# manikya7022/Continual-Learning-for-Dynamic-Video-Quality-Enhancement

Measured on AMD Instinct MI355X. Metric: train frames/sec (2x SR, T=3, 540p->1080p), higher is better.
Workload: dtype bf16

## Files before the change

### continual-learning-for-dynamic-video-quality-enhancement_amd/csrc/conv_bf16.hip

```cpp
#include "conv_common.h"

namespace nvq {

#ifdef NVQ_DEBUG_TOOLS
static int g_debug_mode = 0;
void set_conv_debug_mode(int m) { g_debug_mode = m; }
#else
constexpr int g_debug_mode = 0;
#endif

constexpr int XSB = 48;

__device__ __forceinline__ __bf16 pack_bf16_elem(const float* __restrict__ w, int cout_w, int cin_w, int taps, int transpose,
                                                 int cout_keep, int NT, int nkc, long idx) {
    const int stride = ws_stride_halfs(taps, NT);
    long t = idx % stride;
    const long slab = idx / stride;
    if (t >= (long)taps * 4 * NT * 8) return (__bf16)0.f;
    const int j = t & 7; t >>= 3;
    const int n = t % NT; t /= NT;
    const int g = t & 3; t >>= 2;
    const int tap = (int)t;
    const int kc = slab % nkc;
    const int cz = (int)(slab / nkc);
    const int co = cz * NT + n;
    const int ch = kc * KCB + 8 * g + j;
    float v = 0.f;
    if (!transpose) {
        if (co < cout_w && ch < cin_w) v = w[((long)co * cin_w + ch) * taps + tap];
    } else {
        if (co < cout_keep && ch < cout_w) v = w[((long)ch * cin_w + co) * taps + (taps - 1 - tap)];
    }
    return (__bf16)v;
}

__global__ void pack_bf16_kernel(const float* __restrict__ w, int cout_w, int cin_w, int taps, int transpose,
                                 int cout_keep, int NT, int ncz, int nkc, __bf16* __restrict__ wp) {
    const long total = (long)ncz * nkc * ws_stride_halfs(taps, NT);
    for (long idx = blockIdx.x * (long)blockDim.x + threadIdx.x; idx < total; idx += (long)gridDim.x * blockDim.x)
        wp[idx] = pack_bf16_elem(w, cout_w, cin_w, taps, transpose, cout_keep, NT, nkc, idx);
}

__global__ void pack_batch_bf16_kernel(const PackJobTable t) {
    const PackJobDev j = t.j[blockIdx.y];
    __bf16* wp = reinterpret_cast<__bf16*>(j.wp);
    for (long idx = blockIdx.x * (long)blockDim.x + threadIdx.x; idx < j.total; idx += (long)gridDim.x * blockDim.x)
        wp[idx] = pack_bf16_elem(j.w, j.cout_w, j.cin_w, j.taps, j.transpose, j.cout_keep, j.NT, j.nkc, idx);
}

struct TailArgs {
    const float* frames;
    float* out;
    unsigned char* pass;
    int T, t_center, Cimg;
};
__device__ __forceinline__ float tcc1(float x) { const float A = -0.75f; return ((A + 2.f) * x - (A + 3.f)) * x * x + 1.f; }
__device__ __forceinline__ float tcc2(float x) { const float A = -0.75f; return ((A * x - 5.f * A) * x + 8.f * A) * x - 4.f * A; }
__device__ __forceinline__ void tail_cubic_taps(int dst, float scale, int size, int idx[4], float w[4]) {
    const float real = scale * ((float)dst + 0.5f) - 0.5f;
    const float fl = floorf(real);
    const float t = real - fl;
    const int i0 = (int)fl;
    w[0] = tcc2(t + 1.f);
    w[1] = tcc1(t);
    w[2] = tcc1(1.f - t);
    w[3] = tcc2((1.f - t) + 1.f);
#pragma unroll
    for (int k = 0; k < 4; ++k) idx[k] = min(max(i0 - 1 + k, 0), size - 1);
}

template <int NB, int KS, bool INB, int NW = 4, int CS = 1, int TS = 0>
__global__ __launch_bounds__(64 * NW, NW == 4 ? 2 : 4) void conv_bf16_kernel(const nvq_conv_desc d, int tilesX,
                                                                               int tilesY, int nkc, int vec_ok, int dbg,
                                                                               const TailArgs tail) {
    constexpr int NT = NB * 16;
    constexpr int NTW = NT * CS;
    constexpr int NTHR = 64 * NW;
    constexpr int TH_ = 2 * NW / CS;
    constexpr int HALO = KS / 2;
    constexpr int TAPS = KS * KS;
    constexpr int HW_ = TW + 2 * HALO;
    constexpr int HH_ = TH_ + 2 * HALO;
    constexpr int NPIX = HW_ * HH_;
    constexpr int WS_HALFS = ws_stride_halfs(TAPS, NTW);
    constexpr int XITEMS = NPIX * 4;
    constexpr int XPER = (XITEMS + NTHR - 1) / NTHR;
    constexpr int WTHR = NTHR;
    constexpr int WPIECES = TAPS * 4 * NTW;
    constexpr int WPER = (WPIECES + WTHR - 1) / WTHR;
    constexpr int XREGS = INB ? 1 : 2;
    constexpr int CT_K = (TAPS / 2) * 4 * NTW / WTHR;
    constexpr int CT_N = 4 * NTW;
    static_assert(((TAPS / 2) * 4 * NTW) % WTHR == 0 && CT_N <= 256, "the centre tap starts a WTHR-piece row");
    static_assert(CS == 1 || (CS == 2 && NW == 8 && NB == 2), "channel-split variant: 8 waves, 2 x 32 channels");

    __shared__ __attribute__((aligned(16))) __bf16 lds[NPIX * XSB + WS_HALFS];
    __bf16* xs = lds;
    __bf16* ws = lds + NPIX * XSB;
    const int kcl = KS == 3 ? d.center_cin / KCB : 0;

    const int tid = threadIdx.x;
    const int lane = tid & 63;
    const int wid = __builtin_amdgcn_readfirstlane(tid >> 6);
    const int wave = CS == 1 ? wid : wid & (NW / CS - 1);
    const int half = CS == 1 ? 0 : wid >> 2;
    const int c = lane & 15;
    const int g = lane >> 4;

    int bt = xcd_tile(blockIdx.x, gridDim.x);
    const int tx = bt % tilesX; bt /= tilesX;
    const int ty = bt % tilesY;
    const int n = bt / tilesY;
    const int cz = blockIdx.y * CS + half;
    const int H = d.h, W = d.w;

    f32x4 acc[NB][4];
#pragma unroll
    for (int a = 0; a < NB; ++a)
#pragma unroll
        for (int b = 0; b < 4; ++b) acc[a][b] = (f32x4){0.f, 0.f, 0.f, 0.f};

    const __bf16* wp_base = reinterpret_cast<const __bf16*>(d.wpack) + (size_t)blockIdx.y * nkc * WS_HALFS;
    const float* in32 = d.in + d.in_coff;
    const __bf16* in16 = reinterpret_cast<const __bf16*>(d.in) + d.in_coff;

    unsigned xoff[XPER];
    bool xok[XPER];
#pragma unroll
    for (int k = 0; k < XPER; ++k) {
        const int item = tid + k * NTHR;
        const int hp = item >> 2;
        const int hy = hp / HW_, hx = hp - hy * HW_;
        const int gy = ty * TH_ + hy - HALO, gx = tx * TW + hx - HALO;
        xok[k] = item < XITEMS && gy >= 0 && gy < H && gx >= 0 && gx < W;
        xoff[k] = xok[k] ? (unsigned)(((size_t)(n * H + gy) * W + gx) * (d.in_plane ? 32 : d.in_ld)) : 0u;
    }
    const int nk0 = d.in_plane ? d.in_ld >> 5 : 0x7fffffff;
    const int sh0 = d.in_plane ? __ffs(d.in_ld >> 5) - 1 : 0;
    const bool interior = ty * TH_ >= HALO && tx * TW >= HALO && ty * TH_ + TH_ + HALO <= H && tx * TW + TW + HALO <= W &&
                          d.cin % KCB == 0;
    const int chg = 8 * (tid & 3);
    u32x4 xr[XPER][XREGS];
    u32x4 wr[WPER];

    bool cv0 = false, cv1 = false;
    auto fetch = [&](int kc, bool light) {
        const int ch = kc * KCB + chg;
        cv0 = ch < d.cin;
        cv1 = ch + 4 < d.cin;
        const bool lead = kc < nk0;
        const int sh = lead ? sh0 : 0;
        const unsigned cbase = lead ? (unsigned)kc * KCB : (unsigned)kc * d.in_plane;
        const unsigned o0 = cv0 ? cbase + chg : 0u, o1 = cv1 ? cbase + chg + 4 : 0u;
#pragma unroll
        for (int k = 0; k < XPER; ++k) {
            if constexpr (INB) {
                xr[k][0] = *reinterpret_cast<const u32x4*>(in16 + ((xoff[k] << sh) + o0));
            } else {
                xr[k][0] = *reinterpret_cast<const u32x4*>(in32 + ((xoff[k] << sh) + o0));
                xr[k][XREGS - 1] = *reinterpret_cast<const u32x4*>(in32 + ((xoff[k] << sh) + o1));
            }
        }
        const u32x4* wsrc = reinterpret_cast<const u32x4*>(wp_base + (size_t)kc * WS_HALFS);
        if (light) {
            wr[CT_K] = wsrc[(tid < CT_N ? tid : 0) + CT_K * WTHR];
        } else {
#pragma unroll
            for (int k = 0; k < WPER; ++k) wr[k] = wsrc[tid + k * WTHR < WPIECES ? tid + k * WTHR : 0];
        }
    };
    auto commit = [&](int kc, bool light) {
        const u32x4 z = {0u, 0u, 0u, 0u};
        if (interior) {
#pragma unroll
            for (int k = 0; k < XPER; ++k) {
                const int item = tid + k * NTHR;
                if (item < XITEMS) {
                    __bf16* dst = xs + (item >> 2) * XSB + 8 * (item & 3);
                    if constexpr (INB) *reinterpret_cast<u32x4*>(dst) = xr[k][0];
                    else *reinterpret_cast<bf16x8*>(dst) = cvt8(as_f4(xr[k][0]), as_f4(xr[k][XREGS - 1]));
                }
            }
        } else {
#pragma unroll
            for (int k = 0; k < XPER; ++k) {
                const int item = tid + k * NTHR;
                const bool v0 = xok[k] && cv0, v1 = xok[k] && cv1;
                if (item < XITEMS) {
                    __bf16* dst = xs + (item >> 2) * XSB + 8 * (item & 3);
                    if constexpr (INB)
                        *reinterpret_cast<u32x4*>(dst) = v0 ? xr[k][0] : z;
                    else
                        *reinterpret_cast<bf16x8*>(dst) = cvt8(as_f4(v0 ? xr[k][0] : z), as_f4(v1 ? xr[k][XREGS - 1] : z));
                }
            }
        }
        if (light) {
            if (tid < CT_N) reinterpret_cast<u32x4*>(ws)[tid + CT_K * WTHR] = wr[CT_K];
        } else {
#pragma unroll
            for (int k = 0; k < WPER; ++k)
                if ((k + 1) * WTHR <= WPIECES || tid + k * WTHR < WPIECES) reinterpret_cast<u32x4*>(ws)[tid + k * WTHR] = wr[k];
        }
    };

    auto ldP = [&](int rr, int xh, int dx) -> bf16x8 {
        return *reinterpret_cast<const bf16x8*>(xs + ((2 * wave + rr) * HW_ + xh * 16 + c + dx) * XSB + 8 * g);
    };
    auto ldW = [&](int tap, int cb) -> bf16x8 {
        return *reinterpret_cast<const bf16x8*>(ws + ((tap * 4 + g) * NTW + half * NT + cb * 16 + c) * 8);
    };
    auto stage_chunk = [&](int kc, bool cl, bool fl) {
        __syncthreads();
        commit(kc, cl);
        __syncthreads();
        if (kc + 1 < nkc && !(dbg & 2)) fetch(kc + 1, fl);
    };
    auto center_stage = [&]() {
        bf16x8 p0[2], p1[2], wc[NB];
#pragma unroll
        for (int cb = 0; cb < NB; ++cb) wc[cb] = ldW(TAPS / 2, cb);
#pragma unroll
        for (int xh = 0; xh < 2; ++xh) { p0[xh] = ldP(1, xh, 1); p1[xh] = ldP(2, xh, 1); }
#pragma unroll
        for (int xh = 0; xh < 2; ++xh)
#pragma unroll
            for (int cb = 0; cb < NB; ++cb) {
                acc[cb][xh] = __builtin_amdgcn_mfma_f32_16x16x32_bf16(wc[cb], p0[xh], acc[cb][xh], 0, 0, 0);
                acc[cb][2 + xh] = __builtin_amdgcn_mfma_f32_16x16x32_bf16(wc[cb], p1[xh], acc[cb][2 + xh], 0, 0, 0);
            }
    };

    const bool dead = CS == 2 && cz * NT >= d.cout_store;
    int kc = 0;
    if constexpr (KS == 3) {
        if (kcl > 0) {
            fetch(0, true);
            for (; kc + 1 < kcl; ++kc) {
                stage_chunk(kc, true, true);
                if (!(dbg & 1) && !dead) center_stage();
            }
            stage_chunk(kc, true, false);
            if (!(dbg & 1) && !dead) center_stage();
            ++kc;
        } else {
            fetch(0, false);
        }
    } else {
        fetch(0, false);
    }
    for (; kc < nkc; ++kc) {
        stage_chunk(kc, false, false);
        if ((dbg & 1) || dead) continue;
        bf16x8 lo[2], hi[2], wa[NB], wn[NB];
        lo[0] = ldP(0, 0, 0); lo[1] = ldP(0, 1, 0);
#pragma unroll
        for (int cb = 0; cb < NB; ++cb) wa[cb] = ldW(0, cb);
        hi[0] = ldP(1, 0, 0); hi[1] = ldP(1, 1, 0);
#pragma unroll
        for (int s = 0; s < TAPS; ++s) {
            const int dy = s % KS;
            const bool last = s + 1 == TAPS;
            const int ndx = (s + 1) / KS, ndy = (s + 1) % KS;
            const bool same_dx = !last && ndy != 0;
            bf16x8 nlo[2], nhi[2];
            if (!last) {
#pragma unroll
                for (int cb = 0; cb < NB; ++cb) wn[cb] = ldW(ndy * KS + ndx, cb);
            }
#pragma unroll
            for (int xh = 0; xh < 2; ++xh) {
#pragma unroll
                for (int cb = 0; cb < NB; ++cb)
                    acc[cb][xh] = __builtin_amdgcn_mfma_f32_16x16x32_bf16(wa[cb], lo[xh], acc[cb][xh], 0, 0, 0);
                if (same_dx) nhi[xh] = ldP(dy + 2, xh, ndx);
                else if (!last) nlo[xh] = ldP(0, xh, ndx);
            }
#pragma unroll
            for (int xh = 0; xh < 2; ++xh) {
#pragma unroll
                for (int cb = 0; cb < NB; ++cb)
                    acc[cb][2 + xh] = __builtin_amdgcn_mfma_f32_16x16x32_bf16(wa[cb], hi[xh], acc[cb][2 + xh], 0, 0, 0);
                if (same_dx) nlo[xh] = hi[xh];
                else if (!last) nhi[xh] = ldP(1, xh, ndx);
            }
            if (!last) {
#pragma unroll
                for (int xh = 0; xh < 2; ++xh) { lo[xh] = nlo[xh]; hi[xh] = nhi[xh]; }
#pragma unroll
                for (int cb = 0; cb < NB; ++cb) wa[cb] = wn[cb];
            }
        }
    }
    if constexpr (TS > 0) {
        static_assert(NW == 4 && CS == 1, "8 x 32-pixel tiles");
        constexpr int CP = NT + 1;
        static_assert(TH * TW * CP * 4 <= (NPIX * XSB + WS_HALFS) * 2, "the conv output tile fits the LDS stages");
        float* ut = reinterpret_cast<float*>(lds);
        const int U = tail.Cimg * TS * TS;
        __syncthreads();
#pragma unroll
        for (int pb = 0; pb < 4; ++pb) {
            const int px = (2 * wave + (pb >> 1)) * TW + (pb & 1) * 16 + c;
#pragma unroll
            for (int cb = 0; cb < NB; ++cb)
#pragma unroll
                for (int e = 0; e < 4; ++e) {
                    const int co = cb * 16 + 4 * g + e;
                    if (co < U) ut[px * CP + co] = acc[cb][pb][e] + (d.bias ? d.bias[co] : 0.f);
                }
        }
        __syncthreads();
        const int OW = W * TS, OH = H * TS;
        const float scale = 1.f / (float)TS;
// ... 452 lines not shown
    const __bf16* r16 = reinterpret_cast<const __bf16*>(dl.res) + dl.res_coff;
    auto res_load = [&](int pb) {
        const int gy = ty * TH + 2 * w4 + (pb >> 1), gx = tx * TW + (pb & 1) * 16 + c;
        okp[pb] = gy < H && gx < W;
        const unsigned off = okp[pb] ? ((unsigned)(n * H + gy) * (unsigned)W + gx) * (unsigned)dl.res_ld + 4u * g : 0u;
#pragma unroll
        for (int cb = 0; cb < NBL; ++cb) rr[pb][cb] = *reinterpret_cast<const uint2*>(r16 + (off + cb * 16u));
    };
    if (!(dbg & 128)) { res_load(0); res_load(1); }
    __syncthreads();
    __syncthreads();
    {
        const __bf16* t4 = ws;
#pragma unroll
        for (int cb = 0; cb < NBL; ++cb) {
            const bf16x8 wf = ldL(cb);
#pragma unroll
            for (int pb = 0; pb < 4; ++pb) {
                const int px = (2 * w4 + (pb >> 1)) * TW + (pb & 1) * 16 + c;
                const bf16x8 yf = *reinterpret_cast<const bf16x8*>(t4 + px * T4S + 8 * g);
                lacc[cb][pb] = __builtin_amdgcn_mfma_f32_16x16x32_bf16(wf, yf, lacc[cb][pb], 0, 0, 0);
            }
        }
    }
    if (!(dbg & 128)) { res_load(2); res_load(3); }
#pragma unroll
    for (int cb = 0; cb < NBL; ++cb) bb[cb] = ld4(dl.bias + cb * 16 + 4 * g);
    __syncthreads();
    __bf16* stage = lds + w4 * (2 * TW * STAGE_PX64);
#pragma unroll
    for (int pb = 0; pb < 4; ++pb) {
        if (!okp[pb]) continue;
#pragma unroll
        for (int cb = 0; cb < NBL; ++cb) {
            float v[4] = {lacc[cb][pb][0] + bb[cb].x, lacc[cb][pb][1] + bb[cb].y, lacc[cb][pb][2] + bb[cb].z,
                          lacc[cb][pb][3] + bb[cb].w};
            {
#pragma clang fp contract(off)
                v[0] = v[0] * dl.alpha + __uint_as_float(rr[pb][cb].x << 16);
                v[1] = v[1] * dl.alpha + __uint_as_float(rr[pb][cb].x & 0xffff0000u);
                v[2] = v[2] * dl.alpha + __uint_as_float(rr[pb][cb].y << 16);
                v[3] = v[3] * dl.alpha + __uint_as_float(rr[pb][cb].y & 0xffff0000u);
            }
            *reinterpret_cast<bf16x4*>(stage + ((pb >> 1) * TW + (pb & 1) * 16 + c) * STAGE_PX64 + cb * 16 + 4 * g) =
                (bf16x4){(__bf16)v[0], (__bf16)v[1], (__bf16)v[2], (__bf16)v[3]};
        }
    }
    __builtin_amdgcn_fence(__ATOMIC_RELEASE, "wavefront");
    __builtin_amdgcn_wave_barrier();
    if (dbg & 16) return;
    __bf16* o16 = reinterpret_cast<__bf16*>(dl.out);
#pragma unroll
    for (int k = 0; k < 8; ++k) {
        const int item = lane + k * 64;
        const int px = item >> 3, piece = item & 7;
        const int gy = ty * TH + 2 * w4 + (px >> 5), gx = tx * TW + (px & 31);
        if (gy < H && gx < W)
            *reinterpret_cast<u32x4*>(o16 + ((size_t)(n * H + gy) * W + gx) * dl.out_ld + dl.out_coff + 8 * piece) =
                *reinterpret_cast<const u32x4*>(stage + px * STAGE_PX64 + 8 * piece);
    }
}

template <int KS, bool XB, bool YB, int CIC, int COC = 32>
__global__ __launch_bounds__(256, 2) void wgrad_bf16_kernel(const nvq_wgrad_desc d, int tilesX, int tilesY,
                                                             int ntiles, int nci32, int nco) {
    static_assert(CIC == 32 || (CIC == 64 && XB), "64-channel chunks need bf16 x");
    static_assert(COC == 32 || (COC == 64 && CIC == 64 && YB && KS == 1), "64-co chunks: 1x1, bf16 x and dy");
    constexpr int HALO = KS / 2;
    constexpr int TAPS = KS * KS;
    constexpr int HW_ = TW + 2 * HALO;
    constexpr int HH_ = TH + 2 * HALO;
    constexpr int NPIX = HW_ * HH_;
    constexpr int XSX = CIC == 64 ? 80 : XSB;
    constexpr int XPP = (XB ? 4 : 8) * (CIC / 32);
    constexpr int YSX = COC == 64 ? 80 : XSB;
    constexpr int YPP = (YB ? 4 : 8) * (COC / 32);
    constexpr int XCH = CIC / XPP, YCH = COC / YPP;
    constexpr int XITEMS = NPIX * XPP;
    constexpr int XPER = (XITEMS + 255) / 256;
    constexpr int YPER = TH * TW * YPP / 256;
    constexpr int NCO = (CIC == 64 ? 2 : 1) * (COC / 32);
    __shared__ __attribute__((aligned(16))) __bf16 lds[NPIX * XSX + TH * TW * YSX];
    __bf16* xs = lds;
    __bf16* dys = lds + NPIX * XSX;

    const int tid = threadIdx.x;
    const int lane = tid & 63;
    const int wave = tid >> 6;
    const int r = lane & 15;
    const int g = lane >> 4;
    const int q = r >> 2, p = r & 3;
    const int cib = CIC == 64 ? wave : wave >> 1;
    const int cob0 = CIC == 64 ? 0 : (wave & 1);
    const int cic = blockIdx.y, coc = blockIdx.z;
    const int H = d.h, W = d.w;
    const float* x32 = d.x + d.x_coff;
    const __bf16* x16 = reinterpret_cast<const __bf16*>(d.x) + d.x_coff;
    const float* dy32 = d.dy + d.dy_coff;
    const __bf16* dy16 = reinterpret_cast<const __bf16*>(d.dy) + d.dy_coff;

    f32x4 acc[NCO][TAPS];
#pragma unroll
    for (int a = 0; a < NCO; ++a)
#pragma unroll
        for (int t = 0; t < TAPS; ++t) acc[a][t] = (f32x4){0.f, 0.f, 0.f, 0.f};

    u32x4 xr[XPER], yr[YPER];
    float4 bsumA = make_float4(0.f, 0.f, 0.f, 0.f), bsumB = bsumA;
    const int xq = XCH * (tid & (XPP - 1));
    const int yq = YCH * (tid & (YPP - 1));
    const bool xch_ok = cic * CIC + xq < d.cin;
    const int xch = cic * CIC + xq;
    const bool xlead = !d.x_plane || xch < d.x_ld;
    const unsigned xmul = xlead ? d.x_ld : 32;
    const size_t xbase = xlead ? (size_t)xch : (size_t)(xch >> 5) * d.x_plane + (xch & 31);
    const int ych = coc * COC + yq;
    const bool ych_ok = ych < d.cout;
    unsigned xmask = 0, ymask = 0;
    auto fetch = [&](int tile) {
        int bt = xcd_tile(tile, ntiles);
        const int tx = bt % tilesX; bt /= tilesX;
        const int ty = bt % tilesY;
        const int n = bt / tilesY;
        xmask = 0; ymask = 0;
#pragma unroll
        for (int k = 0; k < XPER; ++k) {
            const int item = tid + k * 256;
            const int hp = item / XPP;
            const int hy = hp / HW_, hx = hp - hy * HW_;
            const int gy = ty * TH + hy - HALO, gx = tx * TW + hx - HALO;
            const bool ok = item < XITEMS && gy >= 0 && gy < H && gx >= 0 && gx < W && xch_ok;
            xmask |= (ok ? 1u : 0u) << k;
            const size_t off = ok ? ((size_t)(n * H + gy) * W + gx) * xmul + xbase : 0;
            if constexpr (XB) xr[k] = *reinterpret_cast<const u32x4*>(x16 + off);
            else xr[k] = *reinterpret_cast<const u32x4*>(x32 + off);
        }
#pragma unroll
        for (int k = 0; k < YPER; ++k) {
            const int item = tid + k * 256;
            const int pp = item / YPP;
            const int py = pp / TW, px = pp - py * TW;
            const int gy = ty * TH + py, gx = tx * TW + px;
            const bool ok = gy < H && gx < W && ych_ok;
            ymask |= (ok ? 1u : 0u) << k;
            const size_t off = ok ? ((size_t)(n * H + gy) * W + gx) * d.dy_ld + ych : 0;
            if constexpr (YB) yr[k] = *reinterpret_cast<const u32x4*>(dy16 + off);
            else yr[k] = *reinterpret_cast<const u32x4*>(dy32 + off);
        }
    };
    auto commit = [&]() {
        const u32x4 z = {0u, 0u, 0u, 0u};
#pragma unroll
        for (int k = 0; k < XPER; ++k) {
            const int item = tid + k * 256;
            if (item < XITEMS) {
                const u32x4 v = (xmask >> k) & 1 ? xr[k] : z;
                __bf16* dst = xs + (item / XPP) * XSX + XCH * (item & (XPP - 1));
                if constexpr (XB) *reinterpret_cast<u32x4*>(dst) = v;
                else *reinterpret_cast<bf16x4*>(dst) = cvt4(as_f4(v));
            }
        }
#pragma unroll
        for (int k = 0; k < YPER; ++k) {
            const int item = tid + k * 256;
            const u32x4 v = (ymask >> k) & 1 ? yr[k] : z;
            __bf16* dst = dys + (item / YPP) * YSX + YCH * (item & (YPP - 1));
            if constexpr (YB) {
                *reinterpret_cast<u32x4*>(dst) = v;
                bsumA.x += bf_lo(v[0]); bsumA.y += bf_hi(v[0]); bsumA.z += bf_lo(v[1]); bsumA.w += bf_hi(v[1]);
                bsumB.x += bf_lo(v[2]); bsumB.y += bf_hi(v[2]); bsumB.z += bf_lo(v[3]); bsumB.w += bf_hi(v[3]);
            } else {
                const float4 f = as_f4(v);
                *reinterpret_cast<bf16x4*>(dst) = cvt4(f);
                bsumA.x += f.x; bsumA.y += f.y; bsumA.z += f.z; bsumA.w += f.w;
            }
        }
    };
    const bool idle = cic * CIC + cib * 16 >= d.cin_w;
    typedef s16x4 __attribute__((address_space(3))) * lds_s16x4_ptr;
    auto tr_read = [&](const __bf16* base, int stride, int pix, int chblock) -> s16x4 {
        return __builtin_amdgcn_ds_read_tr16_b64_v4i16((lds_s16x4_ptr)(base + (pix + q) * stride + chblock * 16 + 4 * p));
    };

    int tile = blockIdx.x;
    if (tile < ntiles) fetch(tile);
    for (; tile < ntiles; tile += gridDim.x) {
        __syncthreads();
        commit();
        __syncthreads();
        if (tile + (int)gridDim.x < ntiles) fetch(tile + gridDim.x);
        if (idle) continue;
#pragma unroll 2
        for (int py = 0; py < TH; ++py) {
            bf16x8 bfrag[NCO];
#pragma unroll
            for (int a = 0; a < NCO; ++a) {
                const s16x4 b0 = tr_read(dys, YSX, py * TW + 4 * g, cob0 + a);
                const s16x4 b1 = tr_read(dys, YSX, py * TW + 16 + 4 * g, cob0 + a);
                bfrag[a] = __builtin_bit_cast(bf16x8, __builtin_shufflevector(b0, b1, 0, 1, 2, 3, 4, 5, 6, 7));
            }
#pragma unroll
            for (int tap = 0; tap < TAPS; ++tap) {
                const int ddy = tap / KS, ddx = tap - ddy * KS;
                const int hp = (py + ddy) * HW_ + ddx;
                const s16x4 a0 = tr_read(xs, XSX, hp + 4 * g, cib);
                const s16x4 a1 = tr_read(xs, XSX, hp + 16 + 4 * g, cib);
                const bf16x8 afrag = __builtin_bit_cast(bf16x8, __builtin_shufflevector(a0, a1, 0, 1, 2, 3, 4, 5, 6, 7));
#pragma unroll
                for (int a = 0; a < NCO; ++a)
                    acc[a][tap] = __builtin_amdgcn_mfma_f32_16x16x32_bf16(afrag, bfrag[a], acc[a][tap], 0, 0, 0);
            }
        }
    }

    const int slab = cic * (CIC / 32) + (cib * 16) / 32;
    if (slab < nci32) {
        const int cil0 = (cib * 16) % 32;
#pragma unroll
        for (int a = 0; a < NCO; ++a) {
            const int coc32 = coc * (COC / 32) + (cob0 + a) / 2, cob = (cob0 + a) % 2;
            if (coc32 >= nco) continue;
            float* part = d.workspace + ((size_t)(blockIdx.x * nci32 + slab) * nco + coc32) * (TAPS * WG_C * WG_C);
#pragma unroll
            for (int tap = 0; tap < TAPS; ++tap)
#pragma unroll
                for (int e = 0; e < 4; ++e) part[(tap * WG_C + cil0 + 4 * g + e) * WG_C + cob * 16 + r] = acc[a][tap][e];
        }
    }

    if (cic == 0 && d.dbias != nullptr) {
        float* scratch = reinterpret_cast<float*>(lds);
        __syncthreads();
        st4(scratch + 8 * tid, bsumA);
        st4(scratch + 8 * tid + 4, bsumB);
        __syncthreads();
        if (tid < COC) {
            const int piece = tid / YCH, e = tid % YCH;
            float s = 0.f;
            for (int k = 0; k < 256 / YPP; ++k) s += scratch[8 * (YPP * k + piece) + e];
            float* bp = d.workspace + (size_t)WGRAD_MAX_SLABS * 9 * WG_C * WG_C;
            const int coc32 = coc * (COC / 32) + tid / WG_C;
            if (coc32 < nco) bp[((size_t)blockIdx.x * nco + coc32) * WG_C + tid % WG_C] = s;
        }
    }
}

size_t pack_floats_bf16(int cout, int cin_store, int ksize) {
    const int NT = choose_nt(cout);
    const size_t ncz = (cout + NT - 1) / NT, nkc = (cin_store + KCB - 1) / KCB;
    return ncz * nkc * (size_t)ws_stride_halfs(ksize * ksize, NT) / 2;
}

int pack_bf16(const float* w, int cout_w, int cin_w, int ksize, int transpose, int cin_store, int cout_keep,
              float* wpack, hipStream_t s) {
    const int cout = transpose ? cout_keep : cout_w;
    const int NT = choose_nt(cout);
    const int ncz = (cout + NT - 1) / NT, nkc = (cin_store + KCB - 1) / KCB;
    const long total = (long)ncz * nkc * ws_stride_halfs(ksize * ksize, NT);
    int nblk = ceil_div(total, 256);
    if (nblk > 2048) nblk = 2048;
    hipLaunchKernelGGL(pack_bf16_kernel, dim3(nblk), dim3(256), 0, s, w, cout_w, cin_w, ksize * ksize, transpose,
                       cout_keep, NT, ncz, nkc, reinterpret_cast<__bf16*>(wpack));
    return check_launch("conv_pack_bf16");
}

PackJobDev pack_job_bf16(const nvq_pack_job& j) {
    const int cout = j.transpose ? j.cout_keep : j.cout_w;
    const int NT = choose_nt(cout);
    const int ncz = (cout + NT - 1) / NT, nkc = (j.cin_store + KCB - 1) / KCB;
    return PackJobDev{j.w, j.wpack, j.cout_w, j.cin_w, j.ksize * j.ksize, j.transpose, j.cout_keep, NT, ncz, nkc,
                      (long)ncz * nkc * ws_stride_halfs(j.ksize * j.ksize, NT)};
}

int pack_batch_bf16(const PackJobTable& t, int n, hipStream_t s) {
    hipLaunchKernelGGL(pack_batch_bf16_kernel, dim3(32, n), dim3(256), 0, s, t);
    return check_launch("conv_pack_batch(bf16)");
}

int conv_forward_bf16(const nvq_conv_desc& d, int vec_ok, hipStream_t s) {
    NVQ_REQUIRE((size_t)d.n * d.h * d.w * d.in_ld < ((size_t)1 << 32),
                "conv_forward(bf16): input tensor of %d x %d x %d x %d elements exceeds the 32-bit offsets of the kernels", d.n,
                d.h, d.w, d.in_ld);
    const int NT = choose_nt(d.cout);
    const int ncz = (d.cout_store + NT - 1) / NT;
    const int nkc = (d.cin + KCB - 1) / KCB;
    int tilesX = (d.w + TW - 1) / TW, tilesY = (d.h + TH - 1) / TH;
    const bool underfilled = tilesX * ((d.h + 2 * TH - 1) / (2 * TH)) < NVQ_SMALL_IMAGE_TILES;
    const int rows = d.tile_rows == 0 && underfilled ? 8 : d.tile_rows;
    if (d.ksize == 3 && NT == 32 && d.in_bf16 && d.h >= 2 * TH && vec_ok &&
        (rows == 162 || rows == 164 || (rows == 0 && d.cin <= 128)))
        return conv_forward_m32(d, rows == 164 ? 4 : 2, g_debug_mode & 15, s);
    if (d.ksize == 3 && NT == 32 && d.in_bf16 && d.h >= 2 * TH && rows != 8) {
        tilesY = (d.h + 2 * TH - 1) / (2 * TH);
        const dim3 grid8((unsigned)((long)tilesX * tilesY * d.n), ncz);
        hipLaunchKernelGGL((conv_bf16_kernel<2, 3, true, 8>), grid8, dim3(512), 0, s, d, tilesX, tilesY, nkc, vec_ok,
                           g_debug_mode & 3, TailArgs{});
        return check_launch("conv_forward_bf16");
    }
    if (d.ksize == 3 && NT == 64 && d.in_bf16 && (d.tile_rows == 264 || d.tile_rows == 265)) {
        NVQ_REQUIRE(vec_ok && d.out_bf16 && d.cout_store % 64 == 0 && d.cin % 8 == 0,
                    "conv_forward: tile_rows 264 / 265 need bf16 output and a multiple of 64 stored channels");
        return conv_forward_m32(d, d.tile_rows == 264 ? 64 : 65, g_debug_mode & 3, s);
    }
    if (d.ksize == 3 && NT == 64 && d.in_bf16 && d.tile_rows != 8) {
        const dim3 grid8((unsigned)((long)tilesX * tilesY * d.n), ncz);
        hipLaunchKernelGGL((conv_bf16_kernel<2, 3, true, 8, 2>), grid8, dim3(512), 0, s, d, tilesX, tilesY, nkc, vec_ok,
                           g_debug_mode & 3, TailArgs{});
        return check_launch("conv_forward_bf16");
    }
    const dim3 grid((unsigned)((long)tilesX * tilesY * d.n), ncz);
#define NVQ_LAUNCH_CONVB(NB, KS)                                                                                        \
    do {                                                                                                                 \
        if (d.in_bf16)                                                                                                   \
            hipLaunchKernelGGL((conv_bf16_kernel<NB, KS, true>), grid, dim3(256), 0, s, d, tilesX, tilesY, nkc, vec_ok, g_debug_mode & 3, TailArgs{});   \
        else                                                                                                             \
            hipLaunchKernelGGL((conv_bf16_kernel<NB, KS, false>), grid, dim3(256), 0, s, d, tilesX, tilesY, nkc, vec_ok, g_debug_mode & 3, TailArgs{});  \
    } while (0)
    if (d.ksize == 3) {
        if (NT == 16) NVQ_LAUNCH_CONVB(1, 3);
        else if (NT == 32) NVQ_LAUNCH_CONVB(2, 3);
        else NVQ_LAUNCH_CONVB(4, 3);
    } else {
        if (NT == 16) NVQ_LAUNCH_CONVB(1, 1);
        else if (NT == 32) NVQ_LAUNCH_CONVB(2, 1);
        else NVQ_LAUNCH_CONVB(4, 1);
    }
#undef NVQ_LAUNCH_CONVB
    return check_launch("conv_forward_bf16");
}

int upsampler_tail_bf16(const nvq_conv_desc& d, const float* frames, int T, int t_center, int Cimg, int s, float* out,
                        unsigned char* pass, hipStream_t st) {
    NVQ_REQUIRE((size_t)d.n * d.h * d.w * d.in_ld < ((size_t)1 << 32), "upsampler_tail: tensor exceeds 32-bit offsets");
    const int tilesX = (d.w + TW - 1) / TW, tilesY = (d.h + TH - 1) / TH;
    const int nkc = (d.cin + KCB - 1) / KCB;
    const dim3 grid((unsigned)((long)tilesX * tilesY * d.n), 1);
    const TailArgs t{frames, out, pass, T, t_center, Cimg};
    if (s == 2 && Cimg * 4 <= 16)
        hipLaunchKernelGGL((conv_bf16_kernel<1, 3, true, 4, 1, 2>), grid, dim3(256), 0, st, d, tilesX, tilesY, nkc, 0, 0, t);
    else if (s == 3 && Cimg * 9 <= 32)
        hipLaunchKernelGGL((conv_bf16_kernel<2, 3, true, 4, 1, 3>), grid, dim3(256), 0, st, d, tilesX, tilesY, nkc, 0, 0, t);
    else if (s == 4 && Cimg * 16 <= 64)
        hipLaunchKernelGGL((conv_bf16_kernel<4, 3, true, 4, 1, 4>), grid, dim3(256), 0, st, d, tilesX, tilesY, nkc, 0, 0, t);
    else
        NVQ_REQUIRE(false, "upsampler_tail: scale %d with %d image channels", s, Cimg);
    return check_launch("upsampler_tail_forward");
}

void conv_occupancy_bf16(int* out) {
    (void)hipOccupancyMaxActiveBlocksPerMultiprocessor(&out[0], conv_bf16_kernel<2, 3, true, 8>, 512, 0);
    (void)hipOccupancyMaxActiveBlocksPerMultiprocessor(&out[1], conv_bf16_kernel<2, 3, true, 8, 2>, 512, 0);
    (void)hipOccupancyMaxActiveBlocksPerMultiprocessor(&out[2], conv_bf16_kernel<4, 3, true, 4>, 256, 0);
    (void)hipOccupancyMaxActiveBlocksPerMultiprocessor(&out[3], rdb_tail_kernel, 256, 0);
    (void)hipOccupancyMaxActiveBlocksPerMultiprocessor(&out[4], wgrad_bf16_kernel<3, true, true, 64, 32>, 256, 0);
    (void)hipOccupancyMaxActiveBlocksPerMultiprocessor(&out[5], conv_bf16_kernel<2, 3, true, 4>, 256, 0);
}

int rdb_tail_bf16(const nvq_conv_desc& d3, const nvq_conv_desc& dl, int vec3, int vecl, hipStream_t s) {
    NVQ_REQUIRE((size_t)d3.n * d3.h * d3.w * d3.in_ld < ((size_t)1 << 32) &&
                    (!dl.res || (size_t)dl.n * dl.h * dl.w * dl.res_ld < ((size_t)1 << 32)),
                "rdb_tail_forward: tensor exceeds 32-bit offsets");
    const int tilesX = (d3.w + TW - 1) / TW, tilesY = (d3.h + TH - 1) / TH;
    const int nkc = d3.cin / KCB;
    const bool usual = dl.out_bf16 && dl.bias && dl.res && dl.res_bf16 && dl.res_cmax >= 64 && !dl.out2 && !dl.relu && vecl;
    if ((d3.tile_rows & 255) == 4 || !usual)
        hipLaunchKernelGGL(rdb_tail_kernel, dim3((unsigned)((long)tilesX * tilesY * d3.n)), dim3(256), 0, s, d3, dl, tilesX,
                           tilesY, nkc, vec3, vecl);
    else
        hipLaunchKernelGGL(rdb_tail8_kernel, dim3((unsigned)((long)tilesX * tilesY * d3.n)), dim3(512), 0, s, d3, dl, tilesX,
                           tilesY, nkc, vec3, vecl);
    return check_launch("rdb_tail_forward");
}

int conv_wgrad_bf16(const nvq_wgrad_desc& d, int nsplit, int nci, int nco, int tilesX, int tilesY, int ntiles,
                    hipStream_t s) {
    if ((d.variant & 15) != 1 && wgrad_m32_takes(d)) return conv_wgrad_m32(d, s);
    NVQ_REQUIRE((d.variant & 15) != 2, "conv_wgrad: variant 2 (all-input-channel kernel) does not take %d -> %d channels, ksize %d",
                d.cin, d.cout, d.ksize);
    const bool wide = d.x_bf16 && d.dy_bf16 && d.cin_w >= 64;
    const int ncig = wide ? (nci + 1) / 2 : nci;
    if (wide) {
        nsplit = WGRAD_MAX_WG / (ncig * nco);
        if (nsplit < 1) nsplit = 1;
        if (nsplit > ntiles) nsplit = ntiles;
        if (nsplit >= 8) nsplit &= ~7;
    }
    NVQ_REQUIRE((size_t)nsplit * nci * nco * d.ksize * d.ksize <= (size_t)WGRAD_MAX_SLABS * 9,
                "conv_wgrad(bf16): %d splits x %d x %d chunks exceed the workspace", nsplit, nci, nco);
    if (wide && d.ksize == 1 && d.cout >= 64) {
        const int nco64 = (nco + 1) / 2;
        nsplit = WGRAD_MAX_WG / (ncig * nco64);
        const int cap = WGRAD_MAX_SLABS * 9 / (nci * nco * d.ksize * d.ksize);
        if (nsplit > cap) nsplit = cap;
        if (nsplit < 1) nsplit = 1;
        if (nsplit > ntiles) nsplit = ntiles;
        if (nsplit >= 8) nsplit &= ~7;
        NVQ_REQUIRE((size_t)nsplit * nci * nco * d.ksize * d.ksize <= (size_t)WGRAD_MAX_SLABS * 9,
                    "conv_wgrad(bf16, 64 co): %d splits x %d x %d chunks exceed the workspace", nsplit, nci, nco);
        hipLaunchKernelGGL((wgrad_bf16_kernel<1, true, true, 64, 64>), dim3(nsplit, ncig, nco64), dim3(256), 0, s, d, tilesX,
                           tilesY, ntiles, nci, nco);
        return nsplit;
    }
    const dim3 grid(nsplit, ncig, nco);
#define NVQ_LAUNCH_WG(KS, XB, YB, CIC) \
    hipLaunchKernelGGL((wgrad_bf16_kernel<KS, XB, YB, CIC>), grid, dim3(256), 0, s, d, tilesX, tilesY, ntiles, nci, nco)
    if (d.ksize == 3) {
        if (wide) NVQ_LAUNCH_WG(3, true, true, 64);
        else if (d.x_bf16 && d.dy_bf16) NVQ_LAUNCH_WG(3, true, true, 32);
        else if (d.x_bf16) NVQ_LAUNCH_WG(3, true, false, 32);
        else if (d.dy_bf16) NVQ_LAUNCH_WG(3, false, true, 32);
        else NVQ_LAUNCH_WG(3, false, false, 32);
    } else {
        if (wide) NVQ_LAUNCH_WG(1, true, true, 64);
        else if (d.x_bf16 && d.dy_bf16) NVQ_LAUNCH_WG(1, true, true, 32);
        else if (d.x_bf16) NVQ_LAUNCH_WG(1, true, false, 32);
        else if (d.dy_bf16) NVQ_LAUNCH_WG(1, false, true, 32);
        else NVQ_LAUNCH_WG(1, false, false, 32);
    }
#undef NVQ_LAUNCH_WG
    return nsplit;
}

}
```

### continual-learning-for-dynamic-video-quality-enhancement_amd/csrc/conv_common.h

```cpp
#pragma once
#include "common.h"

namespace nvq {

constexpr int TH = 8;
constexpr int TW = 32;
constexpr int NVQ_SMALL_IMAGE_TILES = 32;
constexpr int WG_C = 32;
constexpr int WGRAD_MAX_WG = 512;
constexpr int WGRAD_MAX_SLABS = 1536;

static inline int choose_nt(int cout) { return cout <= 16 ? 16 : (cout <= 32 ? 32 : 64); }

#ifdef NVQ_DEBUG_TOOLS
void set_conv_debug_mode(int m);
#endif
void conv_occupancy_bf16(int* out);

typedef short s16x4 __attribute__((ext_vector_type(4)));
typedef unsigned u32x4 __attribute__((ext_vector_type(4)));

constexpr int KCB = 32;

__host__ __device__ constexpr int ws_stride_halfs(int taps, int NT) { return ((taps * 4 * NT * 8 + 2047) / 2048) * 2048; }

__device__ __forceinline__ float4 as_f4(u32x4 v) {
    return make_float4(__uint_as_float(v[0]), __uint_as_float(v[1]), __uint_as_float(v[2]), __uint_as_float(v[3]));
}
__device__ __forceinline__ bf16x4 cvt4(float4 v) {
    return (bf16x4){(__bf16)v.x, (__bf16)v.y, (__bf16)v.z, (__bf16)v.w};
}
__device__ __forceinline__ bf16x8 cvt8(float4 a, float4 b) {
    return (bf16x8){(__bf16)a.x, (__bf16)a.y, (__bf16)a.z, (__bf16)a.w, (__bf16)b.x, (__bf16)b.y, (__bf16)b.z, (__bf16)b.w};
}
__device__ __forceinline__ float bf_lo(unsigned u) { return __uint_as_float(u << 16); }
__device__ __forceinline__ float bf_hi(unsigned u) { return __uint_as_float(u & 0xffff0000u); }

size_t pack_floats_bf16(int cout, int cin_store, int ksize);
int pack_bf16(const float* w, int cout_w, int cin_w, int ksize, int transpose, int cin_store, int cout_keep,
              float* wpack, hipStream_t s);
struct PackJobDev { const float* w; float* wp; int cout_w, cin_w, taps, transpose, cout_keep, NT, ncz, nkc; long total; };
constexpr int PACK_BATCH = 48;
struct PackJobTable { PackJobDev j[PACK_BATCH]; };
int pack_batch_bf16(const PackJobTable& t, int n, hipStream_t s);
PackJobDev pack_job_bf16(const nvq_pack_job& j);
int conv_forward_bf16(const nvq_conv_desc& d, int vec_ok, hipStream_t s);
int conv_wgrad_bf16(const nvq_wgrad_desc& d, int nsplit, int nci, int nco, int tilesX, int tilesY, int ntiles,
                    hipStream_t s);
int upsampler_tail_bf16(const nvq_conv_desc& d, const float* frames, int T, int t_center, int Cimg, int s, float* out,
                        unsigned char* pass, hipStream_t st);
int rdb_tail_bf16(const nvq_conv_desc& d3, const nvq_conv_desc& dl, int vec3, int vecl, hipStream_t s);
int conv_forward_m32(const nvq_conv_desc& d, int variant, int dbg, hipStream_t s);
void conv_occupancy_m32(int* out);
bool wgrad_m32_takes(const nvq_wgrad_desc& d);
int conv_wgrad_m32(const nvq_wgrad_desc& d, hipStream_t s);

__device__ __forceinline__ void wgrad_bias_partial(const nvq_wgrad_desc& d, float4 bsum, float* lds, int nco, int cic,
                                                   int coc) {
    if (cic != 0 || d.dbias == nullptr) return;
    __syncthreads();
    st4(lds + 4 * threadIdx.x, bsum);
    __syncthreads();
    if (threadIdx.x < 32) {
        const int q = threadIdx.x >> 2, e = threadIdx.x & 3;
        float s = 0.f;
        for (int k = 0; k < 32; ++k) s += lds[4 * (8 * k + q) + e];
        float* bp = d.workspace + (size_t)WGRAD_MAX_SLABS * 9 * WG_C * WG_C;
        bp[((size_t)blockIdx.x * nco + coc) * WG_C + threadIdx.x] = s;
    }
}

constexpr int STAGE_PX = 40;
constexpr int STAGE_PX64 = 72;

typedef unsigned raw4 __attribute__((ext_vector_type(4)));
__device__ __forceinline__ raw4 ld_raw4(const float* base, size_t idx, int is_bf16) {
    raw4 r;
    if (is_bf16) {
        const uint2 t = *reinterpret_cast<const uint2*>(reinterpret_cast<const __bf16*>(base) + idx);
        r[0] = t.x; r[1] = t.y;
    } else {
        r = *reinterpret_cast<const raw4*>(base + idx);
    }
    return r;
}
__device__ __forceinline__ float4 raw4_f(raw4 r, int is_bf16) {
    if (is_bf16)
        return make_float4(__uint_as_float(r[0] << 16), __uint_as_float(r[0] & 0xffff0000u), __uint_as_float(r[1] << 16),
                           __uint_as_float(r[1] & 0xffff0000u));
    return make_float4(__uint_as_float(r[0]), __uint_as_float(r[1]), __uint_as_float(r[2]), __uint_as_float(r[3]));
}

template <int NB, bool FULL = (NB <= 2)>
__device__ __forceinline__ void conv_epilogue(const nvq_conv_desc& d, f32x4 (&acc)[NB][4], int n, int ty, int tx,
                                              int cz, int wave, int c, int g, int vec_ok, int th = TH,
                                              __bf16* stage = nullptr, int stage_px = STAGE_PX, bool barrier = false) {
    constexpr int NT = NB * 16;
    const int H = d.h, W = d.w;
    if (vec_ok) {
        bool okp[4];
        size_t pixv[4];
#pragma unroll
        for (int pb = 0; pb < 4; ++pb) {
            const int gy = ty * th + 2 * wave + (pb >> 1), gx = tx * TW + (pb & 1) * 16 + c;
            okp[pb] = gy < H && gx < W;
            pixv[pb] = okp[pb] ? (size_t)(n * H + gy) * W + gx : 0;
        }
        int cov[NB];
#pragma unroll
        for (int cb = 0; cb < NB; ++cb) cov[cb] = cz * NT + cb * 16 + 4 * g;
        constexpr int CG = FULL ? NB : 1;
        constexpr int RP = FULL ? 4 : 1;
        float4 bias4[CG];
        unsigned bits_in[4];
        raw4 res4[CG][RP], msk4[CG];
        auto bias_load = [&](int cb0) {
#pragma unroll
            for (int k = 0; k < CG; ++k) bias4[k] = ld4(d.bias + (cov[cb0 + k] < d.cout ? cov[cb0 + k] : 0));
        };
        auto res_load = [&](int pb, int cb0, int slot) {
#pragma unroll
            for (int k = 0; k < CG; ++k)
                res4[k][slot] = ld_raw4(d.res, pixv[pb] * d.res_ld + d.res_coff + (cov[cb0 + k] < d.res_cmax ? cov[cb0 + k] : 0),
                                        d.res_bf16);
        };
        const int bw = d.bits_words > 0 ? d.bits_words : 1, wsel = (cz * NT) >> 5;
        if constexpr (NB <= 2) {
            if (d.bits_mode == 2) {
#pragma unroll
                for (int pb = 0; pb < 4; ++pb) bits_in[pb] = d.bits[pixv[pb] * bw + wsel];
            }
        }
        if constexpr (FULL) {
            if (d.bias) bias_load(0);
            if (d.res) {
#pragma unroll
                for (int pb = 0; pb < 4; ++pb) res_load(pb, 0, pb);
            }
        }
        if (barrier) __syncthreads();
#pragma unroll
        for (int pb = 0; pb < 4; ++pb) {
            if (!okp[pb]) continue;
            const size_t pix = pixv[pb];
            unsigned bits_out = 0;
#pragma unroll
            for (int cb = 0; cb < NB; ++cb) {
                const int k = cb % CG;
                if (k == 0) {
                    if constexpr (!FULL) {
                        if (d.bias) bias_load(cb);
                        if (d.res) res_load(pb, cb, 0);
                    }
                    if (d.mask) {
#pragma unroll
                        for (int j = 0; j < CG; ++j) {
                            const bool in = cov[cb + j] >= d.mask_c0 && cov[cb + j] < d.mask_c1;
                            msk4[j] = ld_raw4(d.mask, pix * d.mask_ld + d.mask_coff + (in ? cov[cb + j] : 0), d.mask_bf16);
                        }
                    }
                }
                const int co = cov[cb];
                if (co >= d.cout_store) continue;
                float v[4] = {acc[cb][pb][0], acc[cb][pb][1], acc[cb][pb][2], acc[cb][pb][3]};
                if (d.bias && co < d.cout) {
                    v[0] += bias4[k].x; v[1] += bias4[k].y; v[2] += bias4[k].z; v[3] += bias4[k].w;
                }
                if (d.relu) {
#pragma unroll
                    for (int e = 0; e < 4; ++e) v[e] = fmaxf(v[e], 0.f);
                }
#pragma unroll
                for (int e = 0; e < 4; ++e) v[e] *= d.alpha;
                if (d.out2)
                    stx4(d.out2, pix * d.out2_ld + d.out2_coff + co, d.out2_bf16, make_float4(v[0], v[1], v[2], v[3]));
                if (d.res && co < d.res_cmax) {
                    const float4 r = raw4_f(res4[k][RP == 4 ? pb : 0], d.res_bf16);
                    v[0] += r.x; v[1] += r.y; v[2] += r.z; v[3] += r.w;
                }
                const size_t oi = pix * d.out_ld + d.out_coff + co;
                if (d.accumulate) {
                    const float4 o = ldx4(d.out, oi, d.out_bf16);
                    v[0] += o.x; v[1] += o.y; v[2] += o.z; v[3] += o.w;
                }
                if (d.mask && co >= d.mask_c0 && co < d.mask_c1) {
                    const float4 m = raw4_f(msk4[k], d.mask_bf16);
                    if (!(m.x > 0.f)) v[0] = 0.f;
                    if (!(m.y > 0.f)) v[1] = 0.f;
                    if (!(m.z > 0.f)) v[2] = 0.f;
                    if (!(m.w > 0.f)) v[3] = 0.f;
                }
                if constexpr (NB <= 2) {
                    if (d.bits_mode == 2) {
#pragma unroll
                        for (int e = 0; e < 4; ++e)
                            if (!((bits_in[pb] >> ((co & 31) + e)) & 1u)) v[e] = 0.f;
                    } else if (d.bits_mode == 1) {
#pragma unroll
                        for (int e = 0; e < 4; ++e) bits_out |= (v[e] > 0.f ? 1u : 0u) << ((co & 31) + e);
                    }
                }
                if (stage)
                    *reinterpret_cast<bf16x4*>(stage + ((pb >> 1) * TW + (pb & 1) * 16 + c) * stage_px + co - cz * NT) =
                        (bf16x4){(__bf16)v[0], (__bf16)v[1], (__bf16)v[2], (__bf16)v[3]};
                else
                    stx4(d.out, oi, d.out_bf16, make_float4(v[0], v[1], v[2], v[3]));
            }
            if constexpr (NB <= 2) {
                if (d.bits_mode == 1) {
                    bits_out |= __shfl_xor(bits_out, 16, 64);
                    bits_out |= __shfl_xor(bits_out, 32, 64);
                    if (g == 0) d.bits[pix * bw + wsel] = bits_out;
                }
            }
        }
        return;
    }
#pragma unroll
    for (int pb = 0; pb < 4; ++pb) {
        const int row = 2 * wave + (pb >> 1);
        const int gy = ty * th + row;
        const int gx = tx * TW + (pb & 1) * 16 + c;
        if (gy >= H || gx >= W) continue;
        const size_t pix = (size_t)(n * H + gy) * W + gx;
#pragma unroll
        for (int cb = 0; cb < NB; ++cb) {
            const int co = cz * NT + cb * 16 + 4 * g;
#pragma unroll
            for (int e = 0; e < 4; ++e) {
                const int ce = co + e;
                if (ce >= d.cout_store) continue;
                float x = acc[cb][pb][e];
                if (d.bias && ce < d.cout) x += d.bias[ce];
                if (d.relu) x = fmaxf(x, 0.f);
                x *= d.alpha;
                if (d.out2) d.out2[pix * d.out2_ld + d.out2_coff + ce] = x;
                if (d.res && ce < d.res_cmax) x += d.res[pix * d.res_ld + d.res_coff + ce];
                float* op = d.out + pix * d.out_ld + d.out_coff + ce;
                if (d.accumulate) x += *op;
                if (d.mask && ce >= d.mask_c0 && ce < d.mask_c1 &&
                    !(d.mask[pix * d.mask_ld + d.mask_coff + ce] > 0.f))
                    x = 0.f;
                *op = x;
            }
        }
    }
}

}
```

Measured before the change: 79.54.

## Add split-wave conv kernel with direct global-to-LDS weight DMA for 64-channel convs

Adds a new 3x3 bf16 conv forward kernel for NT=64 layers. Two half-blocks of waves each compute 32 output channels from a shared input tile. Weights are loaded straight into LDS with global_load_lds, bypassing registers, and only the centre-tap weights are loaded for the leading centre-only channel chunks. The new path replaces the previous 8-row kernel for most 64-channel convs, except tile_rows 8 and 262, aiming to cut register pressure and weight-staging cost in exchange for a more complex synchronisation scheme.

```diff
diff --git a/continual-learning-for-dynamic-video-quality-enhancement_amd/csrc/conv_bf16.hip b/continual-learning-for-dynamic-video-quality-enhancement_amd/csrc/conv_bf16.hip
--- a/continual-learning-for-dynamic-video-quality-enhancement_amd/csrc/conv_bf16.hip
+++ b/continual-learning-for-dynamic-video-quality-enhancement_amd/csrc/conv_bf16.hip
@@ -8,8 +8,6 @@
 #else
 constexpr int g_debug_mode = 0;
 #endif
-
-constexpr int XSB = 48;
 
 __device__ __forceinline__ __bf16 pack_bf16_elem(const float* __restrict__ w, int cout_w, int cin_w, int taps, int transpose,
                                                  int cout_keep, int NT, int nkc, long idx) {
@@ -1068,6 +1066,8 @@
                     "conv_forward: tile_rows 264 / 265 need bf16 output and a multiple of 64 stored channels");
         return conv_forward_m32(d, d.tile_rows == 264 ? 64 : 65, g_debug_mode & 3, s);
     }
+    if (d.ksize == 3 && NT == 64 && d.in_bf16 && d.tile_rows != 8 && d.tile_rows != 262)
+        return conv_forward_split_dma(d, tilesX, tilesY, nkc, vec_ok, s);
     if (d.ksize == 3 && NT == 64 && d.in_bf16 && d.tile_rows != 8) {
         const dim3 grid8((unsigned)((long)tilesX * tilesY * d.n), ncz);
         hipLaunchKernelGGL((conv_bf16_kernel<2, 3, true, 8, 2>), grid8, dim3(512), 0, s, d, tilesX, tilesY, nkc, vec_ok,
diff --git a/continual-learning-for-dynamic-video-quality-enhancement_amd/csrc/conv_common.h b/continual-learning-for-dynamic-video-quality-enhancement_amd/csrc/conv_common.h
--- a/continual-learning-for-dynamic-video-quality-enhancement_amd/csrc/conv_common.h
+++ b/continual-learning-for-dynamic-video-quality-enhancement_amd/csrc/conv_common.h
@@ -21,6 +21,7 @@
 typedef unsigned u32x4 __attribute__((ext_vector_type(4)));
 
 constexpr int KCB = 32;
+constexpr int XSB = 48;
 
 __host__ __device__ constexpr int ws_stride_halfs(int taps, int NT) { return ((taps * 4 * NT * 8 + 2047) / 2048) * 2048; }
 
@@ -45,6 +46,7 @@
 int pack_batch_bf16(const PackJobTable& t, int n, hipStream_t s);
 PackJobDev pack_job_bf16(const nvq_pack_job& j);
 int conv_forward_bf16(const nvq_conv_desc& d, int vec_ok, hipStream_t s);
+int conv_forward_split_dma(const nvq_conv_desc& d, int tilesX, int tilesY, int nkc, int vec_ok, hipStream_t s);
 int conv_wgrad_bf16(const nvq_wgrad_desc& d, int nsplit, int nci, int nco, int tilesX, int tilesY, int ntiles,
                     hipStream_t s);
 int upsampler_tail_bf16(const nvq_conv_desc& d, const float* frames, int T, int t_center, int Cimg, int s, float* out,
diff --git a/continual-learning-for-dynamic-video-quality-enhancement_amd/csrc/conv_split_dma.hip b/continual-learning-for-dynamic-video-quality-enhancement_amd/csrc/conv_split_dma.hip
--- /dev/null
+++ b/continual-learning-for-dynamic-video-quality-enhancement_amd/csrc/conv_split_dma.hip
@@ -0,0 +1,231 @@
+#include "conv_common.h"
+
+namespace nvq {
+
+typedef __attribute__((address_space(3))) void* lds_void_ptr;
+typedef const __attribute__((address_space(1))) void* global_void_ptr;
+
+__global__ __launch_bounds__(512, 4) void conv_split_dma_kernel(const nvq_conv_desc d, int tilesX, int tilesY, int nkc,
+                                                                int vec_ok) {
+    constexpr int NB = 2, NT = 32, NTW = 64, NW = 8, NTHR = 512, THT = 8, KS = 3, TAPS = 9;
+    constexpr int HW_ = TW + 2, HH_ = THT + 2, NPIX = HW_ * HH_;
+    constexpr int WS_HALFS = ws_stride_halfs(TAPS, NTW);
+    constexpr int WPIECES = TAPS * 4 * NTW;
+    constexpr int WFULL = WPIECES / NTHR;
+    constexpr int WREST = WPIECES - WFULL * NTHR;
+    constexpr int CT_K = (TAPS / 2) * 4 * NTW / NTHR;
+    constexpr int CT_N = 4 * NTW;
+    constexpr int XITEMS = NPIX * 4;
+    constexpr int XPER = (XITEMS + NTHR - 1) / NTHR;
+    constexpr int SPX = STAGE_PX;
+    static_assert(WPIECES * 16 == WS_HALFS * 2 && WREST % 64 == 0, "whole wave-instructions, no padding");
+    static_assert(((TAPS / 2) * 4 * NTW) % NTHR == 0 && CT_N % 64 == 0, "the centre tap is whole wave-instructions of row CT_K");
+    static_assert(2 * TW * SPX * NW <= NPIX * XSB + WS_HALFS, "the output staging tiles fit the LDS images");
+
+    __shared__ __attribute__((aligned(16))) __bf16 lds[NPIX * XSB + WS_HALFS];
+    __bf16* xs = lds;
+    __bf16* ws = lds + NPIX * XSB;
+    const int kcl = d.center_cin / KCB;
+
+    const int tid = threadIdx.x;
+    const int lane = tid & 63;
+    const int wid = __builtin_amdgcn_readfirstlane(tid >> 6);
+    const int wave = wid & 3;
+    const int half = wid >> 2;
+    const int c = lane & 15;
+    const int g = lane >> 4;
+
+    int bt = xcd_tile(blockIdx.x, gridDim.x);
+    const int tx = bt % tilesX; bt /= tilesX;
+    const int ty = bt % tilesY;
+    const int n = bt / tilesY;
+    const int cz = blockIdx.y * 2 + half;
+    const int H = d.h, W = d.w;
+
+    f32x4 acc[NB][4];
+#pragma unroll
+    for (int a = 0; a < NB; ++a)
+#pragma unroll
+        for (int b = 0; b < 4; ++b) acc[a][b] = (f32x4){0.f, 0.f, 0.f, 0.f};
+
+    const char* wp_base = reinterpret_cast<const char*>(d.wpack) + (size_t)blockIdx.y * nkc * WS_HALFS * 2 + tid * 16;
+    char* ws_wave = reinterpret_cast<char*>(ws) + wid * 1024;
+    const __bf16* in16 = reinterpret_cast<const __bf16*>(d.in) + d.in_coff;
+
+    unsigned xoff[XPER];
+    bool xok[XPER];
+#pragma unroll
+    for (int k = 0; k < XPER; ++k) {
+        const int item = tid + k * NTHR;
+        const int hp = item >> 2;
+        const int hy = hp / HW_, hx = hp - hy * HW_;
+        const int gy = ty * THT + hy - 1, gx = tx * TW + hx - 1;
+        xok[k] = item < XITEMS && gy >= 0 && gy < H && gx >= 0 && gx < W;
+        xoff[k] = xok[k] ? (unsigned)(((size_t)(n * H + gy) * W + gx) * (d.in_plane ? 32 : d.in_ld)) : 0u;
+    }
+    const int nk0 = d.in_plane ? d.in_ld >> 5 : 0x7fffffff;
+    const int sh0 = d.in_plane ? __ffs(d.in_ld >> 5) - 1 : 0;
+    const bool interior = ty * THT >= 1 && tx * TW >= 1 && ty * THT + THT + 1 <= H && tx * TW + TW + 1 <= W && d.cin % KCB == 0;
+    const int chg = 8 * (tid & 3);
+    u32x4 xr[XPER];
+    bool cv0 = false;
+
+    auto fetch_x = [&](int kc) {
+        const int ch = kc * KCB + chg;
+        cv0 = ch < d.cin;
+        const bool lead = kc < nk0;
+        const int sh = lead ? sh0 : 0;
+        const unsigned cbase = lead ? (unsigned)kc * KCB : (unsigned)kc * d.in_plane;
+        const unsigned o0 = cv0 ? cbase + chg : 0u;
+#pragma unroll
+        for (int k = 0; k < XPER; ++k) xr[k] = *reinterpret_cast<const u32x4*>(in16 + ((xoff[k] << sh) + o0));
+    };
+    auto commit_x = [&]() {
+        const u32x4 z = {0u, 0u, 0u, 0u};
+        if (interior) {
+#pragma unroll
+            for (int k = 0; k < XPER; ++k) {
+                const int item = tid + k * NTHR;
+                if (item < XITEMS) *reinterpret_cast<u32x4*>(xs + (item >> 2) * XSB + 8 * (item & 3)) = xr[k];
+            }
+        } else {
+#pragma unroll
+            for (int k = 0; k < XPER; ++k) {
+                const int item = tid + k * NTHR;
+                if (item < XITEMS) *reinterpret_cast<u32x4*>(xs + (item >> 2) * XSB + 8 * (item & 3)) = xok[k] && cv0 ? xr[k] : z;
+            }
+        }
+    };
+    auto dma_w = [&](int kc, bool light) {
+        const char* src = wp_base + (size_t)kc * (WS_HALFS * 2);
+        auto piece = [&](int k) {
+            __builtin_amdgcn_global_load_lds((global_void_ptr)(src + k * NTHR * 16), (lds_void_ptr)(ws_wave + k * NTHR * 16), 16, 0,
+                                             0);
+        };
+        if (light) {
+            if (wid < CT_N / 64) piece(CT_K);
+        } else {
+#pragma unroll
+            for (int k = 0; k < WFULL; ++k) piece(k);
+            if (wid < WREST / 64) piece(WFULL);
+        }
+    };
+    auto stage = [&](int kc, bool light) {
+        __syncthreads();
+        commit_x();
+        dma_w(kc, light);
+        __syncthreads();
+    };
+
+    auto ldP = [&](int rr, int xh, int dx) -> bf16x8 {
+        return *reinterpret_cast<const bf16x8*>(xs + ((2 * wave + rr) * HW_ + xh * 16 + c + dx) * XSB + 8 * g);
+    };
+    auto ldW = [&](int tap, int cb) -> bf16x8 {
+        return *reinterpret_cast<const bf16x8*>(ws + ((tap * 4 + g) * NTW + half * NT + cb * 16 + c) * 8);
+    };
+    auto center_mfma = [&]() {
+        bf16x8 p0[2], p1[2], wc[NB];
+#pragma unroll
+        for (int cb = 0; cb < NB; ++cb) wc[cb] = ldW(TAPS / 2, cb);
+#pragma unroll
+        for (int xh = 0; xh < 2; ++xh) { p0[xh] = ldP(1, xh, 1); p1[xh] = ldP(2, xh, 1); }
+#pragma unroll
+        for (int xh = 0; xh < 2; ++xh)
+#pragma unroll
+            for (int cb = 0; cb < NB; ++cb) {
+                acc[cb][xh] = __builtin_amdgcn_mfma_f32_16x16x32_bf16(wc[cb], p0[xh], acc[cb][xh], 0, 0, 0);
+                acc[cb][2 + xh] = __builtin_amdgcn_mfma_f32_16x16x32_bf16(wc[cb], p1[xh], acc[cb][2 + xh], 0, 0, 0);
+            }
+    };
+    auto full_mfma = [&]() {
+        bf16x8 lo[2], hi[2], wa[NB], wn[NB];
+        lo[0] = ldP(0, 0, 0); lo[1] = ldP(0, 1, 0);
+#pragma unroll
+        for (int cb = 0; cb < NB; ++cb) wa[cb] = ldW(0, cb);
+        hi[0] = ldP(1, 0, 0); hi[1] = ldP(1, 1, 0);
+#pragma unroll
+        for (int s = 0; s < TAPS; ++s) {
+            const int dy = s % KS;
+            const bool last = s + 1 == TAPS;
+            const int ndx = (s + 1) / KS, ndy = (s + 1) % KS;
+            const bool same_dx = !last && ndy != 0;
+            bf16x8 nlo[2], nhi[2];
+            if (!last) {
+#pragma unroll
+                for (int cb = 0; cb < NB; ++cb) wn[cb] = ldW(ndy * KS + ndx, cb);
+            }
+#pragma unroll
+            for (int xh = 0; xh < 2; ++xh) {
+#pragma unroll
+                for (int cb = 0; cb < NB; ++cb)
+                    acc[cb][xh] = __builtin_amdgcn_mfma_f32_16x16x32_bf16(wa[cb], lo[xh], acc[cb][xh], 0, 0, 0);
+                if (same_dx) nhi[xh] = ldP(dy + 2, xh, ndx);
+                else if (!last) nlo[xh] = ldP(0, xh, ndx);
+            }
+#pragma unroll
+            for (int xh = 0; xh < 2; ++xh) {
+#pragma unroll
+                for (int cb = 0; cb < NB; ++cb)
+                    acc[cb][2 + xh] = __builtin_amdgcn_mfma_f32_16x16x32_bf16(wa[cb], hi[xh], acc[cb][2 + xh], 0, 0, 0);
+                if (same_dx) nlo[xh] = hi[xh];
+                else if (!last) nhi[xh] = ldP(1, xh, ndx);
+            }
+            if (!last) {
+#pragma unroll
+                for (int xh = 0; xh < 2; ++xh) { lo[xh] = nlo[xh]; hi[xh] = nhi[xh]; }
+#pragma unroll
+                for (int cb = 0; cb < NB; ++cb) wa[cb] = wn[cb];
+            }
+        }
+    };
+
+    const bool dead = cz * NT >= d.cout_store;
+    fetch_x(0);
+    int kc = 0;
+    for (; kc < kcl && kc + 1 < nkc; ++kc) {
+        stage(kc, true);
+        fetch_x(kc + 1);
+        if (!dead) center_mfma();
+    }
+    for (; kc + 1 < nkc; ++kc) {
+        stage(kc, false);
+        fetch_x(kc + 1);
+        if (!dead) full_mfma();
+    }
+    const bool light = kc < kcl;
+    stage(kc, light);
+    if (!dead) {
+        if (light) center_mfma();
+        else full_mfma();
+    }
+
+    const bool can_stage = d.out_bf16 && vec_ok;
+    if (can_stage && !(d.cout_store - cz * NT >= NT)) __syncthreads();
+    if (can_stage && d.cout_store - cz * NT >= NT) {
+        __bf16* stg = lds + wid * (2 * TW * SPX);
+        conv_epilogue<NB>(d, acc, n, ty, tx, cz, wave, c, g, vec_ok, THT, stg, SPX, true);
+        __builtin_amdgcn_fence(__ATOMIC_RELEASE, "wavefront");
+        __builtin_amdgcn_wave_barrier();
+        __bf16* o16 = reinterpret_cast<__bf16*>(d.out);
+#pragma unroll
+        for (int k = 0; k < NT / 8; ++k) {
+            const int item = lane + k * 64;
+            const int px = item / (NT / 8), pc = item % (NT / 8);
+            const int gy = ty * THT + 2 * wave + (px >> 5), gx = tx * TW + (px & 31);
+            if (gy < H && gx < W)
+                *reinterpret_cast<u32x4*>(o16 + ((size_t)(n * H + gy) * W + gx) * d.out_ld + d.out_coff + cz * NT + 8 * pc) =
+                    *reinterpret_cast<const u32x4*>(stg + px * SPX + 8 * pc);
+        }
+        return;
+    }
+    conv_epilogue<NB>(d, acc, n, ty, tx, cz, wave, c, g, vec_ok, THT);
+}
+
+int conv_forward_split_dma(const nvq_conv_desc& d, int tilesX, int tilesY, int nkc, int vec_ok, hipStream_t s) {
+    const int ncz = (d.cout_store + 63) / 64;
+    hipLaunchKernelGGL(conv_split_dma_kernel, dim3((unsigned)((long)tilesX * tilesY * d.n), ncz), dim3(512), 0, s, d, tilesX,
+                       tilesY, nkc, vec_ok);
+    return check_launch("conv_forward_split_dma");
+}
+
+}
```

Result: no change. 80.03, median of 6 (+0.6%).
